# giolucasd/ssrl-vit-mae-jepa

Measured on AMD Instinct MI355X. Metric: images/sec pretrain step (fwd+bwd+opt), ViT-S/8 96px MAE, 1/2/4/8 MI355X, higher is better.
Workload: dtype bf16; 1 GPU; ViT-S/8 96px MAE (enc 384x12x6h, dec 192x2x6h, mask_ratio 0.75), batch 2000/GPU, full step; global_batch=2000, per_gpu_batch=2000, parallelism=dp1

## Files before the change

### ssrl_vit_mae_jepa_amd/csrc/gemm_mfma.h

```cpp
#pragma once
#include "kernels.h"
#include <type_traits>

namespace mae {

constexpr int MFMA_UNSUPPORTED = -7777;

int mfma_linear_fwd(const bf16* A, const bf16* W, int64_t M, int N, int K, const Epi& epi, hipStream_t s);

int mfma_linear_fwd_v2(const bf16* A, const bf16* W, int64_t M, int N, int K, const Epi& epi, hipStream_t s);

int mfma_linear_fwd_v3(const bf16* A, const bf16* W, int64_t M, int N, int K, const Epi& epi, bool w2, hipStream_t s);

template <int MODE> using EpiMode = std::integral_constant<int, MODE>;
template <class TO> struct OutType { using type = TO; };
template <class SUP, class F>
int dispatch_epi(const Epi& e, F&& f) {
  auto typed = [&](auto mode) -> int {
    constexpr int MODE = decltype(mode)::value;
    if (e.out_dt == MAE_F32) {
      if constexpr (SUP::ok(MODE, true)) return f(mode, OutType<float>{});
    } else {
      if constexpr (SUP::ok(MODE, false)) return f(mode, OutType<bf16>{});
    }
    return MFMA_UNSUPPORTED;
  };
  switch (e.mode) {
    case MAE_EPI_NONE: return typed(EpiMode<MAE_EPI_NONE>{});
    case MAE_EPI_GELU: return typed(EpiMode<MAE_EPI_GELU>{});
    case MAE_EPI_RESID: return typed(EpiMode<MAE_EPI_RESID>{});
    case MAE_EPI_DGELU: return typed(EpiMode<MAE_EPI_DGELU>{});
    case MAE_EPI_GELU_GRAD: return typed(EpiMode<MAE_EPI_GELU_GRAD>{});
    case MAE_EPI_MUL: return typed(EpiMode<MAE_EPI_MUL>{});
    case MAE_EPI_GELU_ACT: return typed(EpiMode<MAE_EPI_GELU_ACT>{});
    default: return MFMA_UNSUPPORTED;
  }
}
struct EpiAll {
  static constexpr bool ok(int mode, bool f32out) { return mode != MAE_EPI_RESID || f32out; }
};

template <class KB, class KN, class... Args>
int launch_bias_pair(bool has_bias, KB with_bias, KN without, int grid, int block, int lds, hipStream_t s, Args... args) {
  auto go = [&](auto kern) -> int {
    MAE_HIP(hipFuncSetAttribute((const void*)kern, hipFuncAttributeMaxDynamicSharedMemorySize, lds));
    hipLaunchKernelGGL(kern, dim3(grid), dim3(block), lds, s, args...);
    MAE_LAUNCH_CHECK();
    return 0;
  };
  return has_bias ? go(with_bias) : go(without);
}

bool prefer_bm192(int64_t M, int N, int margin_pct);

int64_t mfma_wgrad_scratch_bytes(int64_t M, int N, int K);
int mfma_linear_wgrad(const bf16* dY, const bf16* A, int64_t M, int N, int K, float* dW, float* db, void* slab, hipStream_t s);

int64_t mfma_wgrad_pair_scratch_bytes(int64_t M, int N0, int K0, int N1, int K1);
int mfma_linear_wgrad_pair(const bf16* dY0, const bf16* A0, int N0, int K0, float* dW0, float* db0, const bf16* dY1, const bf16* A1,
                           int N1, int K1, float* dW1, float* db1, int64_t M, void* slab, hipStream_t s);

int mfma_attention_fwd(const bf16* qkv, int B, int T, int H, int hd, bf16* out, float* lse, hipStream_t s);
int mfma_attention_bwd(const bf16* qkv, const bf16* out, const bf16* d_out, const float* lse, int B, int T, int H, int hd,
                       bf16* d_qkv, hipStream_t s);

// ... 2 lines not shown
```

### ssrl_vit_mae_jepa_amd/csrc/k_gemm.hip

```cpp
#include "kernels.h"
#include "gemm_mfma.h"
#include <cstdlib>
#include <cstring>

namespace mae {

template <class TO>
struct EpiDev {
  int mode;
  const float* bias;
  const void* aux;
  TO* out;
  TO* out2;
  int64_t ld;
  __device__ __forceinline__ void apply(int64_t m, int n, float acc) const {
    const int64_t o = m * ld + n;
    if (bias) acc += bias[n];
    if (mode == MAE_EPI_NONE) {
      out[o] = from_f<TO>(acc);
    } else if (mode == MAE_EPI_GELU) {
      const TO pre = from_f<TO>(acc);
      out[o] = pre;
      out2[o] = from_f<TO>(gelu_erf(to_f(pre)));
    } else if (mode == MAE_EPI_RESID) {
// ... 59 lines not shown
#pragma unroll
    for (int j = 0; j < 4; ++j) {
      const int gn = n0 + tx * 4 + j;
      if (gn >= N) continue;
      if (ATOMIC) atomicAdd(reinterpret_cast<float*>(epi.out) + gm * epi.ld + gn, acc[i][j]);
      else epi.apply(gm, gn, acc[i][j]);
    }
  }
}

template <class TI, class TO>
static int run_generic(const void* A, int64_t sam, int64_t sak, const void* Bm, int64_t sbk, int64_t sbn, int64_t M, int N,
                       int64_t K, const Epi& e, hipStream_t s) {
  EpiDev<TO> d{e.mode, e.bias, e.aux, (TO*)e.out, (TO*)e.out2, (int64_t)N};
  MAE_REQUIRE(cdiv(M, 64) <= 65535, "gemm: M too large for the fallback kernel grid");
  dim3 grid((unsigned)cdiv(N, 64), (unsigned)cdiv(M, 64), 1);
  hipLaunchKernelGGL((gemm_generic_kernel<TI, TO, false>), grid, dim3(256), 0, s, (const TI*)A, sam, sak, (const TI*)Bm, sbk,
                     sbn, M, N, K, K, d);
  MAE_LAUNCH_CHECK();
  return 0;
}

static int check_epi(const Epi& e, int dt, const char* who) {
  MAE_REQUIRE(e.out, "%s: null output", who);
  MAE_REQUIRE(e.mode >= MAE_EPI_NONE && e.mode <= MAE_EPI_GELU_ACT, "%s: unknown epilogue %d", who, e.mode);
  MAE_REQUIRE((e.mode != MAE_EPI_GELU && e.mode != MAE_EPI_GELU_GRAD) || e.out2, "%s: GELU epilogue needs out2", who);
  MAE_REQUIRE((e.mode != MAE_EPI_RESID && e.mode != MAE_EPI_DGELU && e.mode != MAE_EPI_MUL) || e.aux, "%s: epilogue needs aux", who);
  MAE_REQUIRE(e.mode != MAE_EPI_RESID || e.out_dt == MAE_F32, "%s: RESID epilogue writes fp32", who);
  MAE_REQUIRE(dt == MAE_F32 || dt == MAE_BF16, "%s: bad dtype %d", who, dt);
  MAE_REQUIRE(e.out_dt == MAE_F32 || e.out_dt == MAE_BF16, "%s: bad output dtype %d", who, e.out_dt);
  MAE_REQUIRE(!(dt == MAE_F32 && e.out_dt == MAE_BF16), "%s: fp32 operands with bf16 output unsupported", who);
  return 0;
}

int num_cus() {
  static const int n = [] {
    int dev = 0, cus = 0;
    if (hipGetDevice(&dev) != hipSuccess || hipDeviceGetAttribute(&cus, hipDeviceAttributeMultiprocessorCount, dev) != hipSuccess || cus <= 0) cus = 256;
    return cus;
  }();
  return n;
}

bool prefer_bm192(int64_t M, int N, int margin_pct) {
  static const int force = [] { const char* v = getenv("MAE_NT_BM"); return v ? atoi(v) : 0; }();
  if (force == 192) return true;
  if (force == 256) return false;
  const int64_t t256 = cdiv(M, 256) * (N / 192), t192 = cdiv(M, 192) * (N / 192);
  const int64_t c256 = cdiv(t256, num_cus()) * 256, c192 = cdiv(t192, num_cus()) * 192;
  return c192 * 100 < c256 * margin_pct;
}

struct NtSel { const char* text; int first; bool w2; };
static const NtSel kNtSel[] = {{"v1", 1, false}, {"v2", 2, false}, {"v3", 3, false}, {"v3w2", 3, true}};
static NtSel nt_sel() {
  if (const char* v = getenv("MAE_GEMM_NT"))
    for (const NtSel& n : kNtSel)
      if (!strcmp(v, n.text)) return n;
  return kNtSel[2];
}

int launch_linear_fwd(const void* A, const void* W, int64_t M, int N, int K, int dt, const Epi& e, hipStream_t s) {
  MAE_REQUIRE(A && W && M > 0 && N > 0 && K > 0, "linear_fwd: bad arguments");
  MAE_TRY(check_epi(e, dt, "linear_fwd"));
  if (dt == MAE_BF16) {
    const NtSel sel = nt_sel();
    if (sel.first == 3) {
      const int r3 = mfma_linear_fwd_v3((const bf16*)A, (const bf16*)W, M, N, K, e, sel.w2, s);
      if (r3 != MFMA_UNSUPPORTED) return r3;
    }
    if (sel.first >= 2) {
      const int r2 = mfma_linear_fwd_v2((const bf16*)A, (const bf16*)W, M, N, K, e, s);
      if (r2 != MFMA_UNSUPPORTED) return r2;
    }
    const int r = mfma_linear_fwd((const bf16*)A, (const bf16*)W, M, N, K, e, s);
    if (r != MFMA_UNSUPPORTED) return r;
    if (e.out_dt == MAE_BF16) return run_generic<bf16, bf16>(A, K, 1, W, 1, K, M, N, K, e, s);
    return run_generic<bf16, float>(A, K, 1, W, 1, K, M, N, K, e, s);
  }
  return run_generic<float, float>(A, K, 1, W, 1, K, M, N, K, e, s);
}

int launch_linear_dgrad(const void* dY, const void* W, int64_t M, int N, int K, int dt, const Epi& e, hipStream_t s) {
  MAE_REQUIRE(dY && W && M > 0 && N > 0 && K > 0, "linear_dgrad: bad arguments");
  MAE_TRY(check_epi(e, dt, "linear_dgrad"));
  MAE_REQUIRE(e.mode == MAE_EPI_NONE || e.mode == MAE_EPI_DGELU || e.mode == MAE_EPI_MUL, "linear_dgrad: epilogue must be NONE, DGELU or MUL");
  if (dt == MAE_BF16) {
    if (e.out_dt == MAE_BF16) return run_generic<bf16, bf16>(dY, N, 1, W, K, 1, M, K, N, e, s);
    return run_generic<bf16, float>(dY, N, 1, W, K, 1, M, K, N, e, s);
  }
  return run_generic<float, float>(dY, N, 1, W, K, 1, M, K, N, e, s);
}

constexpr int COLSUM_BLOCKS = 256;

template <class T>
__global__ void __launch_bounds__(256) colsum_kernel(const T* __restrict__ dY, int64_t M, int N, float* __restrict__ partial) {
  __shared__ __attribute__((aligned(16))) float red[4][256];
  const int lane = threadIdx.x & 63, wave = threadIdx.x >> 6;
  const int c = blockIdx.y * 256 + lane * 4;
  f32x4 acc = {0.f, 0.f, 0.f, 0.f};
  if (c < N) {
    for (int64_t r = blockIdx.x * 4ll + wave; r < M; r += (int64_t)gridDim.x * 4) acc += load4(dY + r * N + c);
  }
  store4(&red[wave][lane * 4], acc);
  __syncthreads();
  if (wave == 0 && c < N) {
    acc = load4(&red[0][lane * 4]) + load4(&red[1][lane * 4]) + load4(&red[2][lane * 4]) + load4(&red[3][lane * 4]);
    store4(partial + (int64_t)blockIdx.x * N + c, acc);
  }
}

int64_t linear_wgrad_scratch_bytes(int64_t M, int N, int K) {
  return round_up((int64_t)COLSUM_BLOCKS * N * 4, 256) + mfma_wgrad_scratch_bytes(M, N, K);
}

int64_t linear_wgrad_pair_scratch_bytes(int64_t M, int N0, int K0, int N1, int K1) {
  return std::max(std::max(linear_wgrad_scratch_bytes(M, N0, K0), linear_wgrad_scratch_bytes(M, N1, K1)),
                  mfma_wgrad_pair_scratch_bytes(M, N0, K0, N1, K1));
}
// ... 85 lines not shown
```

### ssrl_vit_mae_jepa_amd/csrc/k_gemm_nt3.hip

```cpp
#include "gemm_dev.cuh"
#include <cstdlib>

namespace mae {

namespace {

constexpr int BK3 = 64;
template <int NI, int MI, int WM>
struct Geo3 {
  static constexpr int WN = WM == 8 ? 1 : 2;
  static constexpr int NWV = WN * WM;
  static constexpr int BN = 16 * NI * WN, BM = 16 * MI * WM;
  static constexpr int ASTG = BM * BK3 * 2, WSTG = BN * BK3 * 2;
  static constexpr int CAP = NWV == 8 ? 160 * 1024 : 80 * 1024;
  static constexpr bool STRIP = NWV == 8;
  static constexpr int TAIL = STRIP ? 2 * BN * 4 : 0;
  static constexpr int SW = 2;
  static constexpr int SA_ = (CAP - TAIL - SW * WSTG) / ASTG;
  static constexpr int SA = SA_ >= 4 ? 4 : SA_;
  static constexpr int A_OFF = 0, W_OFF = SA * ASTG, BIAS_OFF = W_OFF + SW * WSTG;
  static constexpr int LDS = BIAS_OFF + TAIL;
  static constexpr int NA = BM / 8 / NWV, NW = BN / 8 / NWV;
  static constexpr int GPW = NA + NW;
  static constexpr int NBIAS = BN / 64;
  static_assert(SA >= 2 && LDS <= CAP && BM % (8 * NWV) == 0 && BN % (8 * NWV) == 0, "LDS budget / even deal of the pieces over the waves");
};

#ifndef MAE_NT3_STORE
#define MAE_NT3_STORE 0
#endif
template <class V> __device__ __forceinline__ void stream_store(V v, V* p) {
  static_assert(sizeof(V) == 16, "16-byte stores only");
#if MAE_NT3_STORE == 0
  __builtin_nontemporal_store(v, p);
#elif MAE_NT3_STORE == 1
  *p = v;
#elif MAE_NT3_STORE == 2
  asm volatile("global_store_dwordx4 %0, %1, off sc1\n\ts_nop 1" ::"v"(p), "v"(v) : "memory");
#else
  asm volatile("global_store_dwordx4 %0, %1, off sc0 sc1\n\ts_nop 1" ::"v"(p), "v"(v) : "memory");
#endif
}
#ifndef MAE_NT3_PART_STORE
#define MAE_NT3_PART_STORE 2
#endif
template <class V> __device__ __forceinline__ void part_store(V v, V* p) {
#if MAE_NT3_PART_STORE == 1
  *p = v;
#else
  stream_store(v, p);
#endif
}
__device__ __forceinline__ void st8(float* p, const f32x4& a, const f32x4& b) {
#if MAE_NT3_PART_STORE == 2
  *reinterpret_cast<f32x4*>(p) = a;
  *reinterpret_cast<f32x4*>(p + 4) = b;
#else
  part_store(a, reinterpret_cast<f32x4*>(p));
  part_store(b, reinterpret_cast<f32x4*>(p + 4));
#endif
}
__device__ __forceinline__ void st8(bf16* p, const f32x4& a, const f32x4& b) { stream_store(pk8(a, b), reinterpret_cast<bf16x8*>(p)); }

constexpr int kStreamPolicy = MAE_NT3_STORE == 0 ? 2 : (MAE_NT3_STORE == 1 ? 0 : (MAE_NT3_STORE == 2 ? 16 : 17));
template <int POLICY, class V>
__device__ __forceinline__ void bstore16(const V& v, __amdgpu_buffer_rsrc_t rs, uint32_t voff, uint32_t soff) {
  typedef __attribute__((ext_vector_type(4))) unsigned u32x4_;
  static_assert(sizeof(V) == 16, "16-byte stores only");
  __builtin_amdgcn_raw_buffer_store_b128(__builtin_bit_cast(u32x4_, v), rs, (int)(voff + soff), 0, POLICY);
}
__device__ __forceinline__ bf16x8 bload16(__amdgpu_buffer_rsrc_t rs, uint32_t voff, uint32_t soff) {
  return __builtin_bit_cast(bf16x8, __builtin_amdgcn_raw_buffer_load_b128(rs, (int)voff, (int)soff, 0));
}

template <int BANKS>
__device__ __forceinline__ bf16x8 row_merge8(const bf16x8& keep, const bf16x8& from) {
  typedef __attribute__((ext_vector_type(4))) unsigned u32x4_;
  u32x4_ k = __builtin_bit_cast(u32x4_, keep);
  const u32x4_ f = __builtin_bit_cast(u32x4_, from);
#pragma unroll
  for (int i = 0; i < 4; ++i) k[i] = (unsigned)__builtin_amdgcn_update_dpp((int)k[i], (int)f[i], 0x128, 0xf, BANKS, false);
  return __builtin_bit_cast(bf16x8, k);
}

template <int I0, int I1, int MI, int NI>
__device__ __forceinline__ void mfma_range(f32x4 (&acc)[MI][NI], const bf16x8 (&a)[MI], const bf16x8 (&b)[NI]) {
#pragma unroll
  for (int i = I0; i < I1; ++i) acc[i / NI][i % NI] = __builtin_amdgcn_mfma_f32_16x16x32_bf16(b[i % NI], a[i / NI], acc[i / NI][i % NI], 0, 0, 0);
}

template <int I0, int I1, int MI, int NI>
__device__ __forceinline__ void mfma_range_first(f32x4 (&acc)[MI][NI], const bf16x8 (&a)[MI], const bf16x8 (&b)[NI]) {
#pragma unroll
  for (int i = I0; i < I1; ++i) acc[i / NI][i % NI] = __builtin_amdgcn_mfma_f32_16x16x32_bf16(b[i % NI], a[i / NI], f32x4{0.f, 0.f, 0.f, 0.f}, 0, 0, 0);
}

template <int MI, int NI, int GPW>
struct Spread {
  static constexpr int NR = MI + NI, REST = MI * NI - NR;
  static constexpr int lo(int q) { return NR + q * REST / GPW; }
  static constexpr int hi(int q) { return NR + (q + 1) * REST / GPW; }
};

}

template <int MODE, class TO, bool HAS_BIAS, int NI, int MI, int WM>
__global__ void __launch_bounds__((64 * Geo3<NI, MI, WM>::NWV), 2) gemm_nt3_kernel(const bf16* __restrict__ A, const bf16* __restrict__ W, int64_t M, int N, int K,
                                                               const float* __restrict__ bias, const void* __restrict__ aux, TO* __restrict__ out,
                                                               TO* __restrict__ out2, int tiles_m, int tiles_n, int a_nt) {
  using G_ = Geo3<NI, MI, WM>;
  using SP = Spread<MI, NI, G_::GPW>;
  constexpr int BM = G_::BM, BN = G_::BN, ASTG = G_::ASTG, WSTG = G_::WSTG, SA = G_::SA, SW = G_::SW, NA = G_::NA, NW = G_::NW, GPW = G_::GPW;
  constexpr int NJ = NI / 2, NR = MI + NI;
  constexpr bool TWO = MODE == MAE_EPI_GELU_GRAD;
  constexpr bool KEEP = MODE == 77;
  constexpr int STORE8 = sizeof(TO) == 2 ? 1 : 2;
  constexpr int E = MI * NJ * STORE8 * (TWO ? 2 : 1);
  static_assert(SW == 2, "the waits below assume weight pieces one step ahead");
  constexpr int NAF = SA > 2 ? NA : 0;
  extern __shared__ __attribute__((aligned(16))) char smem[];
  const int tid = threadIdx.x, lane = tid & 63;
  const int wave = __builtin_amdgcn_readfirstlane(tid >> 6);
  const int wm = wave / G_::WN, wn = wave % G_::WN;
  constexpr int WROWS = 16 * MI;
  const int fr = lane & 15, fq = lane >> 4;
  const int G = gridDim.x, T = tiles_m * tiles_n;
  const int vb = (int)xcd_remap(blockIdx.x, G);
  const int ntile = (T - vb + G - 1) / G;
  const int nk = K / BK3;
  const uint32_t lds0 = (uint32_t)(uintptr_t)((__attribute__((address_space(3))) char*)smem);
  const uint32_t rowbytes = (uint32_t)K * 2u;

  const i32x4 rsA = make_rsrc(A, (uint32_t)((uint64_t)M * rowbytes));
  const i32x4 rsW = make_rsrc(W, (uint32_t)N * rowbytes);
  const i32x4 rsB = make_rsrc(bias, HAS_BIAS ? (uint32_t)N * 4u : 0u);
  const uint32_t r8 = (uint32_t)lane >> 3;
// ... 314 lines not shown
```

### ssrl_vit_mae_jepa_amd/csrc/k_pixels.hip

```cpp
#include "kernels.h"
#include <cstdlib>

namespace mae {

namespace {

int band_walk_misfit(int C, int img, int p, int n, int px_bytes) {
  if (!(p > 0 && img % p == 0 && p % 4 == 0 && img / p <= 64)) return 1;
  return (int64_t)C * p * img * px_bytes <= 96 * 1024 && n <= 8192 ? 0 : 2;
}


__device__ __forceinline__ void load_band(const uint8_t* __restrict__ images, int64_t b, int ph, int C, int img, int p, uint8_t* band) {
  const int wpr = img >> 2, words = C * p * wpr;
  for (int w = threadIdx.x; w < words; w += 256) {
    const int row = w / wpr, col = w - row * wpr;
    const int c = row / p, py = row - c * p;
    const unsigned* src = reinterpret_cast<const unsigned*>(images + ((b * C + c) * (int64_t)img + (ph * p + py)) * img);
    reinterpret_cast<unsigned*>(band)[w] = src[col];
  }
}
__device__ __forceinline__ void load_band(const float* __restrict__ images, int64_t b, int ph, int C, int img, int p, float* band) {
  const int wpr = img >> 2;
  for (int w = threadIdx.x; w < C * p * wpr; w += 256) {
    const int row = w / wpr, col = w - row * wpr;
    const int c = row / p, py = row - c * p;
    store4(band + row * img + col * 4, load4(images + ((b * C + c) * (int64_t)img + (ph * p + py)) * img + col * 4));
  }
}

template <class I>
__device__ __forceinline__ void band_tokens(const I* __restrict__ tok, int64_t b, int n_tok, int g, int ph, bool with_cls, int* list, int* cnt) {
  for (int j = threadIdx.x; j < n_tok; j += 256) {
    const int t = (int)tok[b * n_tok + j];
    bool mine;
    int pw;
    if (t <= 0 && with_cls) { mine = ph == 0; pw = -1; }
    else {
      const int n = t <= 0 ? 0 : (t - 1 < g * g ? t - 1 : g * g - 1); mine = n / g == ph; pw = n - (n / g) * g;
    }
    if (mine) {
      const int slot = atomicAdd(cnt, 1);
      list[slot] = (j << 8) | (pw & 0xff);
    }
  }
}

__device__ __forceinline__ void sort_band_list(const int* list, int n, int* sorted) {
  for (int i = threadIdx.x; i < n; i += 256) {
    const int v = list[i];
    int rank = 0;
    for (int o = 0; o < n; ++o) rank += list[o] < v;
    sorted[rank] = v;
  }
}

}

template <class T, int VEC>
__global__ void __launch_bounds__(256) gather_patches_kernel(const float* __restrict__ images,
                                                             const int32_t* __restrict__ tok, int64_t rows, int k,
                                                             int C, int img, int p, T* __restrict__ out) {
  const int g = img / p;
  const int pv = p / VEC;
  const int units_per_row = C * p * pv;
  const int64_t total = rows * units_per_row;
  for (int64_t u = blockIdx.x * 256ll + threadIdx.x; u < total; u += (int64_t)gridDim.x * 256) {
    const int64_t r = u / units_per_row;
    int rem = (int)(u - r * units_per_row);
    const int c = rem / (p * pv);
    rem -= c * p * pv;
    const int py = rem / pv;
    const int px = (rem - py * pv) * VEC;
    const int t = tok[r];
    const int64_t b = r / k;
    T* dst = out + r * (int64_t)(C * p * p) + (c * p + py) * p + px;
    if (t <= 0) {
#pragma unroll
      for (int i = 0; i < VEC; ++i) dst[i] = from_f<T>(0.f);
    } else {
      const int n = t - 1, ph = n / g, pw = n - ph * g;
      const float* src = images + ((b * C + c) * (int64_t)img + (ph * p + py)) * img + pw * p + px;
      if (VEC == 4) {
        store4(dst, load4(src));
      } else {
#pragma unroll
        for (int i = 0; i < VEC; ++i) dst[i] = from_f<T>(src[i]);
      }
    }
  }
}

template <class T>
__global__ void __launch_bounds__(256) gather_patches_u8_kernel(const uint8_t* __restrict__ images, const int32_t* __restrict__ tok, int B,
                                                                int k, int C, int img, int p, T* __restrict__ out) {
  extern __shared__ __attribute__((aligned(16))) unsigned lds32[];
  uint8_t* band = reinterpret_cast<uint8_t*>(lds32);
  int* list = reinterpret_cast<int*>(band + C * p * img);
// ... 5 lines not shown
    if (threadIdx.x == 0) cnt = 0;
    __syncthreads();
    load_band(images, b, ph, C, img, p, band);
    band_tokens(tok, b, k, g, ph, true, list, &cnt);
    __syncthreads();
    const int n = cnt;
    for (int it = threadIdx.x; it < n * units; it += 256) {
      const int li = it / units, u = it - li * units;
      const int j = list[li] >> 8, pw = list[li] & 0xff;
      const int c = u / (p * p4), rem = u - c * (p * p4);
      const int py = rem / p4, px = (rem - py * p4) << 2;
      T* dst = out + (b * k + j) * (int64_t)P + (c * p + py) * p + px;
      f32x4 v = {0.f, 0.f, 0.f, 0.f};
      if (pw != 0xff) {
        const unsigned w = *reinterpret_cast<const unsigned*>(band + (c * p + py) * img + pw * p + px);
        v = f32x4{norm_u8(w & 0xff), norm_u8((w >> 8) & 0xff), norm_u8((w >> 16) & 0xff), norm_u8(w >> 24)};
      }
      store4(dst, v);
    }
    __syncthreads();
  }
}

template <class T, bool HAS_GRAD>
__global__ void __launch_bounds__(256) mse_images_kernel(const float* __restrict__ pred,
                                                         const float* __restrict__ images,
                                                         const int32_t* __restrict__ mask32, int64_t rows, int m, int C,
                                                         int img, int p, float gscale, float* __restrict__ partial,
                                                         T* __restrict__ dpred) {
  __shared__ float red[4];
  const int g = img / p, pp = p * p;
  const int64_t total = rows * pp;
  float acc = 0.f;
  for (int64_t u = blockIdx.x * 256ll + threadIdx.x; u < total; u += (int64_t)gridDim.x * 256) {
    const int64_t r = u / pp;
    const int q = (int)(u - r * pp);
    const int py = q / p, px = q - py * p;
    const int64_t b = r / m;
    int n = mask32[r] - 1;
    n = n < 0 ? 0 : (n >= g * g ? g * g - 1 : n);
    const int ph = n / g, pw = n - ph * g;
    const float* src = images + (b * C * (int64_t)img + (ph * p + py)) * img + pw * p + px;
    const int64_t o = r * (int64_t)(pp * C) + q * C;
    for (int c = 0; c < C; ++c) {
      const float d = pred[o + c] - src[(int64_t)c * img * img];
      acc += d * d;
      if (HAS_GRAD) dpred[o + c] = from_f<T>(d * gscale);
    }
  }
  acc = block_sum_256(acc, red);
  if (threadIdx.x == 0) partial[blockIdx.x] = acc;
}

template <class PX, class T, bool HAS_GRAD>
__global__ void __launch_bounds__(256) mse_images_band_kernel(const float* __restrict__ pred, const PX* __restrict__ images,
                                                              const int32_t* __restrict__ mask32, int B, int m, int C, int img, int p,
                                                              float gscale, float* __restrict__ partial, T* __restrict__ dpred) {
  extern __shared__ __attribute__((aligned(16))) unsigned lds32[];
  PX* band = reinterpret_cast<PX*>(lds32);
  int* list = reinterpret_cast<int*>(band + C * p * img);
  int* sorted = list + m;
  __shared__ int cnt;
  __shared__ float red[4];
  const int g = img / p, P = C * p * p, p4 = p >> 2, units = p * p4;
  float acc = 0.f;
  for (int64_t bb = blockIdx.x; bb < (int64_t)B * g; bb += gridDim.x) {
    const int64_t b = bb / g;
    const int ph = (int)(bb - b * g);
    if (threadIdx.x == 0) cnt = 0;
    __syncthreads();
    load_band(images, b, ph, C, img, p, band);
    band_tokens(mask32, b, m, g, ph, false, list, &cnt);
    __syncthreads();
    const int n = cnt;
    sort_band_list(list, n, sorted);
    __syncthreads();
    for (int it = threadIdx.x; it < n * units; it += 256) {
      const int li = it / units, u = it - li * units;
      const int j = sorted[li] >> 8, pw = sorted[li] & 0xff;
      const int py = u / p4, px = (u - py * p4) << 2;
      const int64_t o = (b * m + j) * (int64_t)P + (py * p + px) * C;
      const PX* src = band + py * img + pw * p + px;
      for (int v = 0; v < C; ++v) {
        const f32x4 pr = load4(pred + o + 4 * v);
        f32x4 d;
#pragma unroll
        for (int i = 0; i < 4; ++i) {
          const int e = 4 * v + i, pxi = e / C, c = e - pxi * C;
          d[i] = pr[i] - px_value(src + c * p * img + pxi);
          acc += d[i] * d[i];
        }
        if (HAS_GRAD) store4(dpred + o + 4 * v, d * gscale);
      }
    }
    __syncthreads();
  }
  acc = block_sum_256(acc, red);
  if (threadIdx.x == 0) partial[blockIdx.x] = acc;
}

template <class PX>
static int mse_from_images_band(const float* pred, const PX* images, const int32_t* mask32, int B, int m, int C, int img, int p, float grad_scale,
                         float* loss, void* d_pred, int dpred_dt, float* scratch, hipStream_t s) {
  const int64_t n = (int64_t)B * m * p * p * C;
  const int grid = (int)std::min<int64_t>((int64_t)B * (img / p), 1024);
  const float gs = grad_scale * 2.0f / (float)n;
  const size_t lds = (size_t)C * p * img * sizeof(PX) + (size_t)m * 8;
  MAE_LAUNCH_LOSS(mse_images_band_kernel, (PX,), grid, lds, s, d_pred, dpred_dt, scratch, 1.0f / (float)n, loss, pred, images, mask32, B, m, C, img,
                  p, gs);
  return 0;
}

template <class I>
__global__ void __launch_bounds__(256) patchify_gather_kernel(const float* __restrict__ images,
                                                              const I* __restrict__ mask32, int64_t rows, int m,
                                                              int C, int img, int p, float* __restrict__ target) {
  const int g = img / p, pp = p * p;
  const int64_t total = rows * pp;
  for (int64_t u = blockIdx.x * 256ll + threadIdx.x; u < total; u += (int64_t)gridDim.x * 256) {
    const int64_t r = u / pp;
    const int q = (int)(u - r * pp);
    const int py = q / p, px = q - py * p;
    const int64_t b = r / m;
    int n = (int)mask32[r] - 1;
    n = n < 0 ? 0 : (n >= g * g ? g * g - 1 : n);
    const int ph = n / g, pw = n - ph * g;
    const float* src = images + (b * C * (int64_t)img + (ph * p + py)) * img + pw * p + px;
    float* dst = target + r * (int64_t)(pp * C) + q * C;
    for (int c = 0; c < C; ++c) dst[c] = src[(int64_t)c * img * img];
  }
}

template <class I>
__global__ void __launch_bounds__(256) patchify_gather_u8_kernel(const uint8_t* __restrict__ images, const I* __restrict__ mask, int B, int m,
                                                                 int C, int img, int p, float* __restrict__ target) {
  extern __shared__ __attribute__((aligned(16))) unsigned lds32[];
  uint8_t* band = reinterpret_cast<uint8_t*>(lds32);
  int* list = reinterpret_cast<int*>(band + C * p * img);
  __shared__ int cnt;
  const int g = img / p, P = C * p * p, p4 = p >> 2, units = p * p4;
  for (int64_t bb = blockIdx.x; bb < (int64_t)B * g; bb += gridDim.x) {
    const int64_t b = bb / g;
    const int ph = (int)(bb - b * g);
    if (threadIdx.x == 0) cnt = 0;
    __syncthreads();
    load_band(images, b, ph, C, img, p, band);
    band_tokens(mask, b, m, g, ph, false, list, &cnt);
    __syncthreads();
    const int n = cnt;
    for (int it = threadIdx.x; it < n * units; it += 256) {
      const int li = it / units, u = it - li * units;
      const int j = list[li] >> 8, pw = list[li] & 0xff;
      const int py = u / p4, px = (u - py * p4) << 2;
      const int64_t o = (b * m + j) * (int64_t)P + (py * p + px) * C;
      const uint8_t* src = band + py * img + pw * p + px;
      for (int v = 0; v < C; ++v) {
        f32x4 d;
#pragma unroll
        for (int i = 0; i < 4; ++i) {
          const int e = 4 * v + i, pxi = e / C, c = e - pxi * C;
          d[i] = norm_u8(src[c * p * img + pxi]);
// ... 152 lines not shown
```

Baseline: 90940 images/s.

## Add persistent weight-stationary NT GEMM v4 with full-K W panel in LDS

Adds a new forward linear kernel in which each workgroup loads the entire K-deep weight panel for its N tile into LDS once. It then loops persistently over M slabs, prefetching the next slab's A fragments into registers while the current one computes. The epilogue uses DPP row merges and buffer stores, and an optional cache-keeping store policy applies to small outputs. The kernel becomes the default for specific (mode, tiles_n, K) shape families, which removes per-tile weight reloads and launch overhead. The costs are high register pressure, fixed tile shapes, and a fallback to v3 for anything outside the listed shapes.

New measurement: 91960 images/s (median of 6 runs). 1.01x the previous value.

```diff
diff --git a/ssrl_vit_mae_jepa_amd/csrc/gemm_mfma.h b/ssrl_vit_mae_jepa_amd/csrc/gemm_mfma.h
--- a/ssrl_vit_mae_jepa_amd/csrc/gemm_mfma.h
+++ b/ssrl_vit_mae_jepa_amd/csrc/gemm_mfma.h
@@ -11,6 +11,8 @@
 int mfma_linear_fwd_v2(const bf16* A, const bf16* W, int64_t M, int N, int K, const Epi& epi, hipStream_t s);
 
 int mfma_linear_fwd_v3(const bf16* A, const bf16* W, int64_t M, int N, int K, const Epi& epi, bool w2, hipStream_t s);
+
+int mfma_linear_fwd_v4(const bf16* A, const bf16* W, int64_t M, int N, int K, const Epi& epi, bool force, hipStream_t s);
 
 template <int MODE> using EpiMode = std::integral_constant<int, MODE>;
 template <class TO> struct OutType { using type = TO; };
diff --git a/ssrl_vit_mae_jepa_amd/csrc/gemm_nt_epi.cuh b/ssrl_vit_mae_jepa_amd/csrc/gemm_nt_epi.cuh
--- /dev/null
+++ b/ssrl_vit_mae_jepa_amd/csrc/gemm_nt_epi.cuh
@@ -0,0 +1,34 @@
+#pragma once
+#include "gemm_dev.cuh"
+
+namespace mae {
+
+#ifndef MAE_NT3_STORE
+#define MAE_NT3_STORE 0
+#endif
+#ifndef MAE_NT3_PART_STORE
+#define MAE_NT3_PART_STORE 2
+#endif
+
+constexpr int kStreamPolicy = MAE_NT3_STORE == 0 ? 2 : (MAE_NT3_STORE == 1 ? 0 : (MAE_NT3_STORE == 2 ? 16 : 17));
+template <int POLICY, class V>
+__device__ __forceinline__ void bstore16(const V& v, __amdgpu_buffer_rsrc_t rs, uint32_t voff, uint32_t soff) {
+  typedef __attribute__((ext_vector_type(4))) unsigned u32x4_;
+  static_assert(sizeof(V) == 16, "16-byte stores only");
+  __builtin_amdgcn_raw_buffer_store_b128(__builtin_bit_cast(u32x4_, v), rs, (int)(voff + soff), 0, POLICY);
+}
+__device__ __forceinline__ bf16x8 bload16(__amdgpu_buffer_rsrc_t rs, uint32_t voff, uint32_t soff) {
+  return __builtin_bit_cast(bf16x8, __builtin_amdgcn_raw_buffer_load_b128(rs, (int)voff, (int)soff, 0));
+}
+
+template <int BANKS>
+__device__ __forceinline__ bf16x8 row_merge8(const bf16x8& keep, const bf16x8& from) {
+  typedef __attribute__((ext_vector_type(4))) unsigned u32x4_;
+  u32x4_ k = __builtin_bit_cast(u32x4_, keep);
+  const u32x4_ f = __builtin_bit_cast(u32x4_, from);
+#pragma unroll
+  for (int i = 0; i < 4; ++i) k[i] = (unsigned)__builtin_amdgcn_update_dpp((int)k[i], (int)f[i], 0x128, 0xf, BANKS, false);
+  return __builtin_bit_cast(bf16x8, k);
+}
+
+}
diff --git a/ssrl_vit_mae_jepa_amd/csrc/k_gemm.hip b/ssrl_vit_mae_jepa_amd/csrc/k_gemm.hip
--- a/ssrl_vit_mae_jepa_amd/csrc/k_gemm.hip
+++ b/ssrl_vit_mae_jepa_amd/csrc/k_gemm.hip
@@ -135,20 +135,27 @@
 }
 
 struct NtSel { const char* text; int first; bool w2; };
-static const NtSel kNtSel[] = {{"v1", 1, false}, {"v2", 2, false}, {"v3", 3, false}, {"v3w2", 3, true}};
-static NtSel nt_sel() {
+static const NtSel kNtSel[] = {{"v1", 1, false}, {"v2", 2, false}, {"v3", 3, false}, {"v3w2", 3, true}, {"v4", 4, false}};
+static NtSel nt_sel(bool* named) {
+  *named = true;
   if (const char* v = getenv("MAE_GEMM_NT"))
     for (const NtSel& n : kNtSel)
       if (!strcmp(v, n.text)) return n;
-  return kNtSel[2];
+  *named = false;
+  return kNtSel[4];
 }
 
 int launch_linear_fwd(const void* A, const void* W, int64_t M, int N, int K, int dt, const Epi& e, hipStream_t s) {
   MAE_REQUIRE(A && W && M > 0 && N > 0 && K > 0, "linear_fwd: bad arguments");
   MAE_TRY(check_epi(e, dt, "linear_fwd"));
   if (dt == MAE_BF16) {
-    const NtSel sel = nt_sel();
-    if (sel.first == 3) {
+    bool named = false;
+    const NtSel sel = nt_sel(&named);
+    if (sel.first == 4) {
+      const int r4 = mfma_linear_fwd_v4((const bf16*)A, (const bf16*)W, M, N, K, e, named, s);
+      if (r4 != MFMA_UNSUPPORTED) return r4;
+    }
+    if (sel.first >= 3) {
       const int r3 = mfma_linear_fwd_v3((const bf16*)A, (const bf16*)W, M, N, K, e, sel.w2, s);
       if (r3 != MFMA_UNSUPPORTED) return r3;
     }
diff --git a/ssrl_vit_mae_jepa_amd/csrc/k_gemm_nt3.hip b/ssrl_vit_mae_jepa_amd/csrc/k_gemm_nt3.hip
--- a/ssrl_vit_mae_jepa_amd/csrc/k_gemm_nt3.hip
+++ b/ssrl_vit_mae_jepa_amd/csrc/k_gemm_nt3.hip
@@ -1,4 +1,4 @@
-#include "gemm_dev.cuh"
+#include "gemm_nt_epi.cuh"
 #include <cstdlib>
 
 namespace mae {
@@ -26,9 +26,6 @@
   static_assert(SA >= 2 && LDS <= CAP && BM % (8 * NWV) == 0 && BN % (8 * NWV) == 0, "LDS budget / even deal of the pieces over the waves");
 };
 
-#ifndef MAE_NT3_STORE
-#define MAE_NT3_STORE 0
-#endif
 template <class V> __device__ __forceinline__ void stream_store(V v, V* p) {
   static_assert(sizeof(V) == 16, "16-byte stores only");
 #if MAE_NT3_STORE == 0
@@ -41,9 +38,6 @@
   asm volatile("global_store_dwordx4 %0, %1, off sc0 sc1\n\ts_nop 1" ::"v"(p), "v"(v) : "memory");
 #endif
 }
-#ifndef MAE_NT3_PART_STORE
-#define MAE_NT3_PART_STORE 2
-#endif
 template <class V> __device__ __forceinline__ void part_store(V v, V* p) {
 #if MAE_NT3_PART_STORE == 1
   *p = v;
@@ -61,27 +55,6 @@
 #endif
 }
 __device__ __forceinline__ void st8(bf16* p, const f32x4& a, const f32x4& b) { stream_store(pk8(a, b), reinterpret_cast<bf16x8*>(p)); }
-
-constexpr int kStreamPolicy = MAE_NT3_STORE == 0 ? 2 : (MAE_NT3_STORE == 1 ? 0 : (MAE_NT3_STORE == 2 ? 16 : 17));
-template <int POLICY, class V>
-__device__ __forceinline__ void bstore16(const V& v, __amdgpu_buffer_rsrc_t rs, uint32_t voff, uint32_t soff) {
-  typedef __attribute__((ext_vector_type(4))) unsigned u32x4_;
-  static_assert(sizeof(V) == 16, "16-byte stores only");
-  __builtin_amdgcn_raw_buffer_store_b128(__builtin_bit_cast(u32x4_, v), rs, (int)(voff + soff), 0, POLICY);
-}
-__device__ __forceinline__ bf16x8 bload16(__amdgpu_buffer_rsrc_t rs, uint32_t voff, uint32_t soff) {
-  return __builtin_bit_cast(bf16x8, __builtin_amdgcn_raw_buffer_load_b128(rs, (int)voff, (int)soff, 0));
-}
-
-template <int BANKS>
-__device__ __forceinline__ bf16x8 row_merge8(const bf16x8& keep, const bf16x8& from) {
-  typedef __attribute__((ext_vector_type(4))) unsigned u32x4_;
-  u32x4_ k = __builtin_bit_cast(u32x4_, keep);
-  const u32x4_ f = __builtin_bit_cast(u32x4_, from);
-#pragma unroll
-  for (int i = 0; i < 4; ++i) k[i] = (unsigned)__builtin_amdgcn_update_dpp((int)k[i], (int)f[i], 0x128, 0xf, BANKS, false);
-  return __builtin_bit_cast(bf16x8, k);
-}
 
 template <int I0, int I1, int MI, int NI>
 __device__ __forceinline__ void mfma_range(f32x4 (&acc)[MI][NI], const bf16x8 (&a)[MI], const bf16x8 (&b)[NI]) {
diff --git a/ssrl_vit_mae_jepa_amd/csrc/k_gemm_nt4.hip b/ssrl_vit_mae_jepa_amd/csrc/k_gemm_nt4.hip
--- /dev/null
+++ b/ssrl_vit_mae_jepa_amd/csrc/k_gemm_nt4.hip
@@ -0,0 +1,265 @@
+#include "gemm_nt_epi.cuh"
+#include <cstdlib>
+
+namespace mae {
+
+namespace {
+
+constexpr int BM4 = 256, BN4 = 192, MI4 = 2, NI4 = 12, NWV4 = 8;
+template <int NK>
+struct Geo4 {
+  static constexpr int WSTG = BN4 * 128;
+  static constexpr int BIAS_OFF = NK * WSTG;
+  static constexpr int LDS = BIAS_OFF + BN4 * 4;
+  static constexpr int NC = 2 * NK;
+  static constexpr int PIECES = NK * (BN4 / 8) / NWV4;
+  static_assert(LDS <= 160 * 1024 && (NK * (BN4 / 8)) % NWV4 == 0, "LDS budget / even deal of the panel over the waves");
+};
+constexpr int PRE4 = 4;
+constexpr int DEFER4 = 2;
+
+struct Nt4Family { int mode; bool f32; int tiles_n, K; };
+constexpr Nt4Family kNt4Families[] = {
+    {MAE_EPI_GELU_GRAD, false, 8, 384},
+    {MAE_EPI_GELU_GRAD, false, 4, 192},
+    {MAE_EPI_NONE, false, 6, 384},
+    {MAE_EPI_NONE, false, 3, 192},
+    {MAE_EPI_MUL, false, 8, 384},
+    {MAE_EPI_MUL, false, 4, 192},
+};
+bool nt4_family(int mode, bool f32, int tiles_n, int K) {
+  for (const Nt4Family& f : kNt4Families)
+    if (f.mode == mode && f.f32 == f32 && f.tiles_n == tiles_n && f.K == K) return true;
+  return false;
+}
+
+}
+
+template <int MODE, class TO, bool HAS_BIAS, int NK, bool A_NT>
+__global__ void __launch_bounds__(64 * NWV4, 2) gemm_nt4_kernel(const bf16* __restrict__ A, const bf16* __restrict__ W, int64_t M, int N,
+                                                                const float* __restrict__ bias, const void* __restrict__ aux, TO* __restrict__ out,
+                                                                TO* __restrict__ out2, int tiles_m, int tiles_n) {
+  using G_ = Geo4<NK>;
+  constexpr int MI = MI4, NI = NI4, NJ = NI / 2, NC = G_::NC, WSTG = G_::WSTG;
+  constexpr bool TWO = MODE == MAE_EPI_GELU_GRAD;
+  constexpr bool KEEP = MODE == 77;
+  constexpr uint32_t rowbytes = 128u * NK;
+  extern __shared__ __attribute__((aligned(16))) char smem[];
+  const int tid = threadIdx.x, lane = tid & 63;
+  const int wave = __builtin_amdgcn_readfirstlane(tid >> 6);
+  const int fr = lane & 15, fq = lane >> 4;
+  const int G = gridDim.x;
+  const int vb = (int)xcd_remap(blockIdx.x, G);
+  const int tn = vb % tiles_n, NG = G / tiles_n;
+  const uint32_t lds0 = (uint32_t)(uintptr_t)((__attribute__((address_space(3))) char*)smem);
+
+  const __amdgpu_buffer_rsrc_t rsA = __builtin_amdgcn_make_buffer_rsrc(const_cast<bf16*>(A), 0, (int)(uint32_t)((uint64_t)M * rowbytes), 0x00020000);
+  const uint32_t va = (uint32_t)(wave * (16 * MI) + fr) * rowbytes + (uint32_t)fq * 16u;
+  auto lda = [&](uint32_t so, int c, int mi) -> bf16x8 {
+    return __builtin_bit_cast(bf16x8, __builtin_amdgcn_raw_buffer_load_b128(rsA, (int)(va + (uint32_t)mi * 16u * rowbytes + (uint32_t)c * 64u), (int)so, A_NT ? 2 : 0));
+  };
+  int slab = vb / tiles_n;
+  uint32_t so_a = (uint32_t)slab * BM4 * rowbytes;
+  bf16x8 a[NC][MI];
+#pragma unroll
+  for (int c = 0; c < NC; ++c)
+#pragma unroll
+    for (int mi = 0; mi < MI; ++mi) a[c][mi] = lda(so_a, c, mi);
+
+  {
+    const i32x4 rsW = make_rsrc(W, (uint32_t)N * rowbytes);
+    const uint32_t r8 = (uint32_t)lane >> 3;
+    const uint32_t voff = r8 * rowbytes + ((((uint32_t)lane & 7u) ^ r8) << 4);
+#pragma unroll
+    for (int i = 0; i < G_::PIECES; ++i) {
+      const int p = wave + NWV4 * i, ks = p / (BN4 / 8), grp = p % (BN4 / 8);
+      dma16(rsW, lds0 + (uint32_t)(ks * WSTG + grp * 1024), voff, ((uint32_t)(tn * BN4 + grp * 8)) * rowbytes + (uint32_t)ks * 128u);
+    }
+    if (HAS_BIAS && wave < BN4 / 64) {
+      const i32x4 rsB = make_rsrc(bias, (uint32_t)N * 4u);
+      dma4(rsB, lds0 + (uint32_t)(G_::BIAS_OFF + 256 * wave), (uint32_t)lane * 4u, (uint32_t)(tn * BN4 * 4 + 256 * wave));
+    }
+    asm volatile("s_waitcnt vmcnt(0)" ::: "memory");
+    __syncthreads();
+  }
+
+  const uint32_t out_bytes = (uint32_t)((uint64_t)M * (uint64_t)N * sizeof(TO));
+  const __amdgpu_buffer_rsrc_t rsO = __builtin_amdgcn_make_buffer_rsrc((void*)out, 0, (int)out_bytes, 0x00020000);
+  const __amdgpu_buffer_rsrc_t rsO2 = __builtin_amdgcn_make_buffer_rsrc((void*)(MODE == MAE_EPI_GELU_GRAD ? out2 : out), 0, (int)out_bytes, 0x00020000);
+  const __amdgpu_buffer_rsrc_t rsX = __builtin_amdgcn_make_buffer_rsrc(const_cast<void*>(MODE == MAE_EPI_MUL ? aux : (const void*)out), 0, (int)out_bytes, 0x00020000);
+  const int gb = (fq & 1) ? 3 + fq : fq;
+  const uint32_t vo_one = ((uint32_t)(wave * (16 * MI) + fr) * (uint32_t)N + (uint32_t)(4 * gb)) * (uint32_t)sizeof(TO);
+  const uint32_t vo_pair = ((uint32_t)(wave * (16 * MI) + (fr & 7)) * (uint32_t)N + (uint32_t)(4 * gb + (fr < 8 ? 0 : 32))) * (uint32_t)sizeof(TO);
+  const float* const sbias = reinterpret_cast<const float*>(smem + G_::BIAS_OFF);
+  const int n0 = tn * BN4;
+
+  f32x4 acc[MI][NI];
+  constexpr int DEFER = MODE == MAE_EPI_MUL ? (NC >= 10 ? 5 : 4) : DEFER4;
+  bf16x8 qx[MODE == MAE_EPI_MUL ? MI : 1][NJ];
+  constexpr uint32_t OSZ = sizeof(TO);
+  const uint32_t rowb = (uint32_t)N * OSZ;
+  auto epilogue = [&](uint32_t so_tile) {
+    if constexpr (MODE == MAE_EPI_MUL) {
+#pragma unroll
+      for (int j = 0; j < NJ; ++j) qx[MI - 1][j] = bload16(rsX, vo_one, so_tile + 16u * rowb + (uint32_t)(64 * j));
+    }
+    MAE_REGROUP8(acc, MI, NI)
+    if constexpr (sizeof(TO) == 2) {
+      constexpr int POL = KEEP ? 0 : kStreamPolicy;
+#pragma unroll
+      for (int mi = 0; mi < MI; ++mi) {
+        const uint32_t so = so_tile + (uint32_t)(mi * 16) * rowb;
+#pragma unroll
+        for (int ja = 0; ja < NJ; ja += 2) {
+          bf16x8 pa[2], pb[TWO ? 2 : 1];
+#pragma unroll
+          for (int jj = 0; jj < 2; ++jj) {
+            const int j = ja + jj;
+            const int nl = 32 * j + 4 * gb;
+            f32x4 b0 = {0.f, 0.f, 0.f, 0.f}, b1 = b0;
+            if (HAS_BIAS) { b0 = load4(sbias + nl); b1 = load4(sbias + nl + 4); }
+            f32x4 v0 = acc[mi][2 * j], v1 = acc[mi][2 * j + 1];
+            if (HAS_BIAS) { v0 += b0; v1 += b1; }
+            if (MODE == MAE_EPI_GELU_GRAD || MODE == MAE_EPI_GELU_ACT) {
+              f32x4 a0, a1, g0, g1;
+              gelu_rounded<TO>(v0, v1, a0, a1, g0, g1);
+              if (MODE == MAE_EPI_GELU_GRAD) { pa[jj] = pk8(g0, g1); pb[TWO ? jj : 0] = pk8(a0, a1); }
+              else pa[jj] = pk8(a0, a1);
+            } else if (MODE == MAE_EPI_MUL) {
+              f32x4 q0, q1;
+              unpack8(qx[MODE == MAE_EPI_MUL ? mi : 0][j], q0, q1);
+              pa[jj] = pk8(v0 * q0, v1 * q1);
+            } else {
+              pa[jj] = pk8(v0, v1);
+            }
+          }
+          auto store_rows = [&](__amdgpu_buffer_rsrc_t rs, const bf16x8* pk) {
+            const bf16x8 S1 = row_merge8<0xc>(pk[0], pk[1]), S2 = row_merge8<0x3>(pk[1], pk[0]);
+            bstore16<POL>(S1, rs, vo_pair, so + (uint32_t)(64 * ja));
+            bstore16<POL>(S2, rs, vo_pair, so + (uint32_t)(64 * ja) + 8u * rowb);
+          };
+          store_rows(rsO, pa);
+          if (TWO) store_rows(rsO2, pb);
+        }
+      }
+    } else {
+      constexpr int POLF = MAE_NT3_PART_STORE >= 1 ? 0 : kStreamPolicy;
+#pragma unroll
+      for (int j = 0; j < NJ; ++j) {
+        const int nl = 32 * j + 4 * gb;
+        f32x4 b0 = {0.f, 0.f, 0.f, 0.f}, b1 = b0;
+        if (HAS_BIAS) { b0 = load4(sbias + nl); b1 = load4(sbias + nl + 4); }
+#pragma unroll
+        for (int mi = 0; mi < MI; ++mi) {
+          const uint32_t so = so_tile + (uint32_t)(mi * 16) * rowb + (uint32_t)(128 * j);
+          f32x4 v0 = acc[mi][2 * j], v1 = acc[mi][2 * j + 1];
+          if (HAS_BIAS) { v0 += b0; v1 += b1; }
+          bstore16<POLF>(v0, rsO, vo_one, so);
+          bstore16<POLF>(v1, rsO, vo_one, so + 16u);
+        }
+      }
+    }
+  };
+
+  const char* const rd_w0 = smem + fr * 128 + (((0 + fq) ^ (fr & 7)) << 4);
+  const char* const rd_w1 = smem + fr * 128 + (((4 + fq) ^ (fr & 7)) << 4);
+  auto rdb = [&](int u) -> bf16x8 {
+    const int c = u / NI, ni = u % NI;
+    return *reinterpret_cast<const bf16x8*>(((c & 1) ? rd_w1 : rd_w0) + (c >> 1) * WSTG + ni * 2048);
+  };
+  for (; slab < tiles_m; slab += NG) {
+    const int nslab = slab + NG < tiles_m ? slab + NG : tiles_m;
+    const uint32_t so_n = (uint32_t)nslab * BM4 * rowbytes;
+    const uint32_t so_tile = ((uint32_t)slab * BM4 * (uint32_t)N + (uint32_t)n0) * OSZ;
+    asm volatile("" ::: "memory");
+    bf16x8 bq[PRE4];
+#pragma unroll
+    for (int u = 0; u < PRE4; ++u) bq[u] = rdb(u);
+#pragma unroll
+    for (int c = 0; c < NC; ++c) {
+#pragma unroll
+      for (int ni = 0; ni < NI; ++ni) {
+        const int u = c * NI + ni;
+        const bf16x8 b = bq[u % PRE4];
+        if (u + PRE4 < NC * NI) bq[u % PRE4] = rdb(u + PRE4);
+#pragma unroll
+        for (int mi = 0; mi < MI; ++mi)
+          acc[mi][ni] = __builtin_amdgcn_mfma_f32_16x16x32_bf16(b, a[c][mi], c == 0 ? f32x4{0.f, 0.f, 0.f, 0.f} : acc[mi][ni], 0, 0, 0);
+        if (u + PRE4 < NC * NI) __builtin_amdgcn_sched_group_barrier(0x100, 1, 0);
+        __builtin_amdgcn_sched_group_barrier(0x008, MI, 0);
+      }
+      __builtin_amdgcn_sched_barrier(0);
+      if (c < NC - DEFER) {
+#pragma unroll
+        for (int mi = 0; mi < MI; ++mi) a[c][mi] = lda(so_n, c, mi);
+      }
+      if constexpr (MODE == MAE_EPI_MUL) {
+        if (c >= NC - 4 && c < NC - 1) {
+          const int j = 2 * (c - (NC - 4));
+          qx[0][j] = bload16(rsX, vo_one, so_tile + (uint32_t)(64 * j));
+          qx[0][j + 1] = bload16(rsX, vo_one, so_tile + (uint32_t)(64 * (j + 1)));
+        }
+      }
+      __builtin_amdgcn_sched_barrier(0);
+    }
+    epilogue(so_tile);
+    __builtin_amdgcn_sched_barrier(0);
+#pragma unroll
+    for (int c = NC - DEFER; c < NC; ++c)
+#pragma unroll
+      for (int mi = 0; mi < MI; ++mi) a[c][mi] = lda(so_n, c, mi);
+    __builtin_amdgcn_sched_barrier(0);
+  }
+}
+
+template <int MODE, class TO, int NK>
+static int launch_nt4(const bf16* A, const bf16* W, int64_t M, int N, const Epi& e, int grid, int tiles_m, int tiles_n, hipStream_t s) {
+  using G_ = Geo4<NK>;
+  if (tiles_n == 1)
+    return launch_bias_pair(e.bias != nullptr, gemm_nt4_kernel<MODE, TO, true, NK, true>, gemm_nt4_kernel<MODE, TO, false, NK, true>, grid, 64 * NWV4, G_::LDS, s,
+                            A, W, M, N, e.bias, e.aux, (TO*)e.out, (TO*)e.out2, tiles_m, tiles_n);
+  return launch_bias_pair(e.bias != nullptr, gemm_nt4_kernel<MODE, TO, true, NK, false>, gemm_nt4_kernel<MODE, TO, false, NK, false>, grid, 64 * NWV4, G_::LDS, s,
+                          A, W, M, N, e.bias, e.aux, (TO*)e.out, (TO*)e.out2, tiles_m, tiles_n);
+}
+
+template <int MODE, class TO>
+static int launch_nt4_k(const bf16* A, const bf16* W, int64_t M, int N, int K, const Epi& e, int grid, int tiles_m, int tiles_n, hipStream_t s) {
+  switch (K / 64) {
+    case 3: return launch_nt4<MODE, TO, 3>(A, W, M, N, e, grid, tiles_m, tiles_n, s);
+    case 4: return launch_nt4<MODE, TO, 4>(A, W, M, N, e, grid, tiles_m, tiles_n, s);
+    case 5: return launch_nt4<MODE, TO, 5>(A, W, M, N, e, grid, tiles_m, tiles_n, s);
+    case 6: return launch_nt4<MODE, TO, 6>(A, W, M, N, e, grid, tiles_m, tiles_n, s);
+    default: return MFMA_UNSUPPORTED;
+  }
+}
+
+struct EpiV4 {
+  static constexpr bool ok(int mode, bool f32out) {
+    return mode == MAE_EPI_NONE || (!f32out && (mode == MAE_EPI_GELU_GRAD || mode == MAE_EPI_GELU_ACT || mode == MAE_EPI_MUL));
+  }
+};
+
+int mfma_linear_fwd_v4(const bf16* A, const bf16* W, int64_t M, int N, int K, const Epi& e, bool force, hipStream_t s) {
+  if (K % 64 != 0 || K < 192 || K > 384 || N % BN4 != 0 || M < 1) return MFMA_UNSUPPORTED;
+  if ((((uintptr_t)A | (uintptr_t)W | (uintptr_t)e.out | (uintptr_t)e.out2 | (uintptr_t)e.bias | (uintptr_t)e.aux) & 15) != 0) return MFMA_UNSUPPORTED;
+  if ((uint64_t)(M + 512) * (uint64_t)K * 2u >= (1ull << 32) || (uint64_t)N * (uint64_t)K * 2u >= (1ull << 32)) return MFMA_UNSUPPORTED;
+  if ((uint64_t)(M + 512) * (uint64_t)N * (e.out_dt == MAE_F32 ? 4u : 2u) >= (1ull << 32)) return MFMA_UNSUPPORTED;
+  const int64_t tiles_m64 = cdiv(M, BM4);
+  const int tiles_n = N / BN4;
+  if (tiles_m64 >= (1ll << 24) || tiles_n > num_cus()) return MFMA_UNSUPPORTED;
+  const int tiles_m = (int)tiles_m64;
+  const int groups = std::min(tiles_m, num_cus() / tiles_n);
+  if (!force && (tiles_m < num_cus() / tiles_n || !nt4_family(e.mode, e.out_dt == MAE_F32, tiles_n, K))) return MFMA_UNSUPPORTED;
+  const int grid = groups * tiles_n;
+  return dispatch_epi<EpiV4>(e, [&](auto mode, auto to) {
+    constexpr int MODE = decltype(mode)::value;
+    using TO = typename decltype(to)::type;
+    if constexpr (MODE == MAE_EPI_NONE && sizeof(TO) == 2) {
+      static const int64_t keep = [] { const char* v = getenv("MAE_NT_KEEP"); return v ? atoll(v) : 64ll << 20; }();
+      if (keep > 0 && M * (int64_t)N * 2 <= keep && N % 256 != 0) return launch_nt4_k<77, bf16>(A, W, M, N, K, e, grid, tiles_m, tiles_n, s);
+    }
+    return launch_nt4_k<MODE, TO>(A, W, M, N, K, e, grid, tiles_m, tiles_n, s);
+  });
+}
+
+}
```

## Double-buffer image bands in MSE loss kernel with async global-to-LDS loads

Applied to the files above, without the earlier changes.

Restructures the band-based MSE loss kernel so the next band of image pixels is fetched into a second LDS buffer with global_load_lds while the current band's loss is computed. Token bucketing for the next band is overlapped in the same way. The inner walk is unrolled two ways, batches its pred loads, and replaces per-element divisions with incremental channel offsets. This aims to hide global-memory latency in the loss step, at the cost of doubled LDS use and possibly lower occupancy; a heuristic falls back to the single-buffer path when LDS is insufficient.

New measurement: 89930 images/s before, 90850 images/s after, median of 6. +1.0%, better.

```diff
diff --git a/ssrl_vit_mae_jepa_amd/csrc/k_pixels.hip b/ssrl_vit_mae_jepa_amd/csrc/k_pixels.hip
--- a/ssrl_vit_mae_jepa_amd/csrc/k_pixels.hip
+++ b/ssrl_vit_mae_jepa_amd/csrc/k_pixels.hip
@@ -29,21 +29,49 @@
   }
 }
 
+template <class PX>
+__device__ __forceinline__ void load_band_dma(const PX* __restrict__ images, int64_t b, int ph, int C, int img, int p, PX* band) {
+  constexpr int WB = 4 * (int)sizeof(PX);
+  const int wpr = img >> 2, words = C * p * wpr, lane = threadIdx.x & 63;
+  for (int w0 = __builtin_amdgcn_readfirstlane(threadIdx.x & ~63); w0 < words; w0 += 256) {
+    const int w = w0 + lane;
+    if (w < words) {
+      const int row = w / wpr, col = w - row * wpr;
+      const int c = row / p, py = row - c * p;
+      const PX* src = images + ((b * C + c) * (int64_t)img + (ph * p + py)) * img + col * 4;
+      const auto* gsrc = (const __attribute__((address_space(1))) void*)src;
+      auto* ldst = (__attribute__((address_space(3))) void*)(reinterpret_cast<char*>(band) + w0 * WB);
+      if constexpr (WB == 4) __builtin_amdgcn_global_load_lds(gsrc, ldst, 4, 0, 0);
+      else __builtin_amdgcn_global_load_lds(gsrc, ldst, 16, 0, 0);
+    }
+  }
+}
+
+__device__ __forceinline__ void wait_band_dma() {
+  asm volatile("" ::: "memory");
+  __builtin_amdgcn_s_waitcnt(0x0F70);
+  asm volatile("" ::: "memory");
+}
+
+__device__ __forceinline__ int64_t band_image(int64_t bb, int g, bool small) {
+  return small ? (int64_t)((uint32_t)bb / (uint32_t)g) : bb / g;
+}
+
+__device__ __forceinline__ void band_token(int t, int j, int g, int ph, bool with_cls, int* list, int* cnt) {
+  bool mine;
+  int pw;
+  if (t <= 0 && with_cls) { mine = ph == 0; pw = -1; }
+  else {
+    const int n = t <= 0 ? 0 : (t - 1 < g * g ? t - 1 : g * g - 1); mine = n / g == ph; pw = n - (n / g) * g;
+  }
+  if (mine) {
+    const int slot = atomicAdd(cnt, 1);
+    list[slot] = (j << 8) | (pw & 0xff);
+  }
+}
 template <class I>
-__device__ __forceinline__ void band_tokens(const I* __restrict__ tok, int64_t b, int n_tok, int g, int ph, bool with_cls, int* list, int* cnt) {
-  for (int j = threadIdx.x; j < n_tok; j += 256) {
-    const int t = (int)tok[b * n_tok + j];
-    bool mine;
-    int pw;
-    if (t <= 0 && with_cls) { mine = ph == 0; pw = -1; }
-    else {
-      const int n = t <= 0 ? 0 : (t - 1 < g * g ? t - 1 : g * g - 1); mine = n / g == ph; pw = n - (n / g) * g;
-    }
-    if (mine) {
-      const int slot = atomicAdd(cnt, 1);
-      list[slot] = (j << 8) | (pw & 0xff);
-    }
-  }
+__device__ __forceinline__ void band_tokens(const I* __restrict__ tok, int64_t b, int n_tok, int g, int ph, bool with_cls, int* list, int* cnt, int j0 = 0) {
+  for (int j = j0 + threadIdx.x; j < n_tok; j += 256) band_token((int)tok[b * n_tok + j], j, g, ph, with_cls, list, cnt);
 }
 
 __device__ __forceinline__ void sort_band_list(const int* list, int n, int* sorted) {
@@ -155,51 +183,144 @@
   if (threadIdx.x == 0) partial[blockIdx.x] = acc;
 }
 
-template <class PX, class T, bool HAS_GRAD>
+template <class PX, class T, bool HAS_GRAD, class F>
+__device__ __forceinline__ float band_loss_walk(const float* __restrict__ pred, const PX* band, const int* sorted, int n, int64_t b, int m, int C,
+                                                int img, int p, float gscale, T* __restrict__ dpred, float acc, F after_first_loads) {
+  constexpr int U = 2, CB = 4;
+  const int P = C * p * p, p4 = p >> 2, units = p * p4, total = n * units;
+  const int cstep = p * img, cwrap = C * cstep - 1;
+  auto use = [&](const f32x4& pr, int64_t o, const PX* src, int v, int& c, int& off) {
+    f32x4 d;
+#pragma unroll
+    for (int i = 0; i < 4; ++i) {
+      d[i] = pr[i] - px_value(src + off);
+      acc += d[i] * d[i];
+      off += cstep;
+      if (++c == C) { c = 0; off -= cwrap; }
+    }
+    if (HAS_GRAD) store4(dpred + o + 4 * v, d * gscale);
+  };
+  bool first = true;
+  for (int it0 = threadIdx.x; it0 < total; it0 += U * 256) {
+    int64_t o[U];
+    const PX* src[U];
+    bool live[U];
+#pragma unroll
+    for (int u = 0; u < U; ++u) {
+      const int it = it0 + u * 256;
+      live[u] = it < total;
+      const int itc = live[u] ? it : it0;
+      const int li = itc / units, r = itc - li * units;
+      const int j = sorted[li] >> 8, pw = sorted[li] & 0xff;
+      const int py = r / p4, px = (r - py * p4) << 2;
+      o[u] = (b * m + j) * (int64_t)P + (py * p + px) * C;
+      src[u] = band + py * img + pw * p + px;
+    }
+    if (C <= CB) {
+      f32x4 pr[U][CB];
+#pragma unroll
+      for (int u = 0; u < U; ++u)
+#pragma unroll
+        for (int v = 0; v < CB; ++v)
+          if (live[u] && v < C) pr[u][v] = load4(pred + o[u] + 4 * v);
+      if (first) { after_first_loads(); first = false; }
+#pragma unroll
+      for (int u = 0; u < U; ++u) {
+        int c = 0, off = 0;
+#pragma unroll
+        for (int v = 0; v < CB; ++v)
+          if (live[u] && v < C) use(pr[u][v], o[u], src[u], v, c, off);
+      }
+    } else {
+      if (first) { after_first_loads(); first = false; }
+#pragma unroll
+      for (int u = 0; u < U; ++u)
+        if (live[u]) {
+          int c = 0, off = 0;
+          for (int v = 0; v < C; ++v) use(load4(pred + o[u] + 4 * v), o[u], src[u], v, c, off);
+        }
+    }
+  }
+  if (first) after_first_loads();
+  return acc;
+}
+
+template <bool PIPE, class PX, class T, bool HAS_GRAD>
 __global__ void __launch_bounds__(256) mse_images_band_kernel(const float* __restrict__ pred, const PX* __restrict__ images,
                                                               const int32_t* __restrict__ mask32, int B, int m, int C, int img, int p,
                                                               float gscale, float* __restrict__ partial, T* __restrict__ dpred) {
   extern __shared__ __attribute__((aligned(16))) unsigned lds32[];
+  constexpr int NB = PIPE ? 2 : 1;
+  const int bandpx = C * p * img;
   PX* band = reinterpret_cast<PX*>(lds32);
-  int* list = reinterpret_cast<int*>(band + C * p * img);
-  int* sorted = list + m;
-  __shared__ int cnt;
+  int* list = reinterpret_cast<int*>(band + NB * bandpx);
+  int* sorted = list + NB * m;
+  __shared__ int cnt[2];
   __shared__ float red[4];
-  const int g = img / p, P = C * p * p, p4 = p >> 2, units = p * p4;
+  const int g = img / p;
+  const int64_t nbands = (int64_t)B * g;
   float acc = 0.f;
-  for (int64_t bb = blockIdx.x; bb < (int64_t)B * g; bb += gridDim.x) {
-    const int64_t b = bb / g;
-    const int ph = (int)(bb - b * g);
-    if (threadIdx.x == 0) cnt = 0;
-    __syncthreads();
-    load_band(images, b, ph, C, img, p, band);
-    band_tokens(mask32, b, m, g, ph, false, list, &cnt);
-    __syncthreads();
-    const int n = cnt;
-    sort_band_list(list, n, sorted);
-    __syncthreads();
-    for (int it = threadIdx.x; it < n * units; it += 256) {
-      const int li = it / units, u = it - li * units;
-      const int j = sorted[li] >> 8, pw = sorted[li] & 0xff;
-      const int py = u / p4, px = (u - py * p4) << 2;
-      const int64_t o = (b * m + j) * (int64_t)P + (py * p + px) * C;
-      const PX* src = band + py * img + pw * p + px;
-      for (int v = 0; v < C; ++v) {
-        const f32x4 pr = load4(pred + o + 4 * v);
-        f32x4 d;
-#pragma unroll
-        for (int i = 0; i < 4; ++i) {
-          const int e = 4 * v + i, pxi = e / C, c = e - pxi * C;
-          d[i] = pr[i] - px_value(src + c * p * img + pxi);
-          acc += d[i] * d[i];
-        }
-        if (HAS_GRAD) store4(dpred + o + 4 * v, d * gscale);
-      }
-    }
-    __syncthreads();
+  if constexpr (!PIPE) {
+    for (int64_t bb = blockIdx.x; bb < nbands; bb += gridDim.x) {
+      const int64_t b = bb / g;
+      const int ph = (int)(bb - b * g);
+      if (threadIdx.x == 0) cnt[0] = 0;
+      __syncthreads();
+      load_band(images, b, ph, C, img, p, band);
+      band_tokens(mask32, b, m, g, ph, false, list, &cnt[0]);
+      __syncthreads();
+      const int n = cnt[0];
+      sort_band_list(list, n, sorted);
+      __syncthreads();
+      acc = band_loss_walk<PX, T, HAS_GRAD>(pred, band, sorted, n, b, m, C, img, p, gscale, dpred, acc, [] {});
+      __syncthreads();
+    }
+  } else {
+    const bool small = nbands + gridDim.x < (1ll << 31);
+    if (threadIdx.x < 2) cnt[threadIdx.x] = 0;
+    __syncthreads();
+    {
+      const int64_t b = blockIdx.x / g;
+      const int ph = (int)(blockIdx.x - b * g);
+      load_band_dma(images, b, ph, C, img, p, band);
+      band_tokens(mask32, b, m, g, ph, false, list, &cnt[0]);
+      wait_band_dma();
+    }
+    __syncthreads();
+    int cur = 0;
+    for (int64_t bb = blockIdx.x; bb < nbands; bb += gridDim.x, cur ^= 1) {
+      const int64_t b = band_image(bb, g, small);
+      const int n = cnt[cur];
+      sort_band_list(list + cur * m, n, sorted);
+      __syncthreads();
+      const int nxt = cur ^ 1;
+      const int64_t nbb = bb + gridDim.x, nb = band_image(nbb, g, small);
+      const int nph = (int)(nbb - nb * g);
+      const bool more = nbb < nbands;
+      acc = band_loss_walk<PX, T, HAS_GRAD>(pred, band + cur * bandpx, sorted, n, b, m, C, img, p, gscale, dpred, acc, [&] {
+        int tn = 0;
+        const bool mine = more && (int)threadIdx.x < m;
+        if (more) load_band_dma(images, nb, nph, C, img, p, band + nxt * bandpx);
+        if (mine) tn = mask32[nb * m + threadIdx.x];
+        wait_band_dma();
+        if (mine) band_token(tn, (int)threadIdx.x, g, nph, false, list + nxt * m, &cnt[nxt]);
+      });
+      if (threadIdx.x == 0) cnt[cur] = 0;
+      if (more) band_tokens(mask32, nb, m, g, nph, false, list + nxt * m, &cnt[nxt], 256);
+      __syncthreads();
+    }
   }
   acc = block_sum_256(acc, red);
   if (threadIdx.x == 0) partial[blockIdx.x] = acc;
+}
+
+static size_t band_loss_lds(int C, int img, int p, int m, int px_bytes, int nb) {
+  return (size_t)nb * C * p * img * px_bytes + (size_t)(nb + 1) * m * 4;
+}
+static bool band_loss_pipelined(int C, int img, int p, int m, int px_bytes) {
+  const size_t cu = 160 * 1024, fixed = 64;
+  const size_t one = band_loss_lds(C, img, p, m, px_bytes, 1) + fixed, two = band_loss_lds(C, img, p, m, px_bytes, 2) + fixed;
+  return two <= cu && cu / two >= std::min<size_t>(4, cu / one);
 }
 
 template <class PX>
@@ -208,8 +329,14 @@
   const int64_t n = (int64_t)B * m * p * p * C;
   const int grid = (int)std::min<int64_t>((int64_t)B * (img / p), 1024);
   const float gs = grad_scale * 2.0f / (float)n;
-  const size_t lds = (size_t)C * p * img * sizeof(PX) + (size_t)m * 8;
-  MAE_LAUNCH_LOSS(mse_images_band_kernel, (PX,), grid, lds, s, d_pred, dpred_dt, scratch, 1.0f / (float)n, loss, pred, images, mask32, B, m, C, img,
+  if (band_loss_pipelined(C, img, p, m, (int)sizeof(PX))) {
+    const size_t lds = band_loss_lds(C, img, p, m, (int)sizeof(PX), 2);
+    MAE_LAUNCH_LOSS(mse_images_band_kernel, (true, PX,), grid, lds, s, d_pred, dpred_dt, scratch, 1.0f / (float)n, loss, pred, images, mask32, B, m, C,
+                    img, p, gs);
+    return 0;
+  }
+  const size_t lds = band_loss_lds(C, img, p, m, (int)sizeof(PX), 1);
+  MAE_LAUNCH_LOSS(mse_images_band_kernel, (false, PX,), grid, lds, s, d_pred, dpred_dt, scratch, 1.0f / (float)n, loss, pred, images, mask32, B, m, C, img,
                   p, gs);
   return 0;
 }
```
